# avianphysics/avian

Hardware: NVIDIA H100
Metric: physics steps/sec on 100k-cube stack (broad phase + solver stage per step) (higher is better)
Workload: dtype f32

## Files before the change

avian_b200/csrc/solver_dev.cuh:

```cuda
#pragma once
#include <cuda_pipeline.h>

#include "../../include/avian_b200.h"
#include "avn_math.cuh"

namespace avn {

enum { CP_N = 0, CP_T1 = 1, CP_TV = 2, CP_IDX = 3, CP_PT0 = 4, CP_PLANES = CP_PT0 + 3 * AVN_MAX_MANIFOLD_POINTS };
#define CP_ROW(k, r) (CP_PT0 + 3 * (k) + (r))
enum { CI_NP_MASK = 0x7, CI_ZERO1 = 1 << 4, CI_ZERO2 = 1 << 5, CI_NONDYN = 1 << 6, CI_TANGENT = 1 << 7,
       CI_VER1 = 1 << 8, CI_VER2 = 1 << 9,
       CI_FIV1 = 1 << 10, CI_FIV2 = 1 << 11,
       CI_FIP1 = 1 << 12, CI_FIP2 = 1 << 13 };
enum { BF_LOCK_MASK = 0x3f, BF_HAS_SOLVER_BODY = 1 << 8, BF_KINEMATIC = 1 << 9, BF_GYRO = 1 << 10, BF_DYNAMIC = 1 << 11,
       BF_CUSTOM_VEL = 1 << 12, BF_CUSTOM_POS = 1 << 13, BF_FUSE_IV = 1 << 14, BF_FUSE_IP = 1 << 15, BF_DOMINANCE_SHIFT = 16 };

enum { JP_IDX = 0,
       JP_R1 = 1,
       JP_R2 = 2,
       JP_CD = 3,
       JP_RD = 4,
       JP_A1 = 5,
       JP_A2 = 6,
       JP_B1 = 7,
// ... 193 lines not shown
    {
        S rcp = S(1) / len(tvv);
        if (avn_finite(rcp) && rcp > S(0)) t1 = tvv * rcp; else t1 = any_orthonormal(fd);
    }
    V3<S> t2 = cross(fd, t1);
    S friction = d.m_friction[m], restitution = d.m_restitution[m];
    if (friction > S(0)) info |= CI_TANGENT;
    if (restitution != S(0)) *d.any_restitution = 1;
    V3<S> tv = ldv3_or0(d.m_tanvel, m);
    st4(&c[CP_N * MP], mk4<S>(n.x, n.y, n.z, friction));
    st4(&c[CP_T1 * MP], mk4<S>(t1.x, t1.y, t1.z, restitution));
    st4(&c[CP_TV * MP], mk4<S>(tv.x, tv.y, tv.z, S(0)));
    st4(&c[CP_IDX * MP], mk4<S>(int_as(S(0), b1), int_as(S(0), b2), int_as(S(0), info), int_as(S(0), 0)));
    bool warm = d.match_contacts != 0;
    for (int k = 0; k < np; ++k) {
        uint32_t p = p0 + k;
        V3<S> r1 = ldv3(d.p_anchor1, p), r2 = ldv3(d.p_anchor2, p);
        V3<S> r1xn = cross(r1, n), r2xn = cross(r2, n);
        S k_linear = dot(n, cmul(mass_sum, n));
        S kk = k_linear + dot(r1xn, smul(in1.ii, r1xn)) + dot(r2xn, smul(in2.ii, r2xn));
        S meff = recip_or_zero(kk);
        S sep0 = -d.p_penetration[p] - dot(r2 - r1, n);
        S imp_n = warm ? d.p_ws_normal[p] : S(0);
        S itx = S(0), ity = S(0), K1 = S(0), K2 = S(0), K3 = S(0);
        if (info & CI_TANGENT) {
            if (warm) { itx = d.p_ws_tangent[2 * p]; ity = d.p_ws_tangent[2 * p + 1]; }
            V3<S> rt11 = cross(r1, t1), rt12 = cross(r2, t1), rt21 = cross(r1, t2), rt22 = cross(r2, t2);
            V3<S> i1_rt11 = smul(in1.ii, rt11), i2_rt12 = smul(in2.ii, rt12), i1_rt21 = smul(in1.ii, rt21), i2_rt22 = smul(in2.ii, rt22);
            S kl1 = dot(t1, cmul(mass_sum, t1)), kl2 = dot(t2, cmul(mass_sum, t2));
            K1 = kl1 + dot(rt11, i1_rt11) + dot(rt12, i2_rt12);
            K2 = kl2 + dot(rt21, i1_rt21) + dot(rt22, i2_rt22);
            K3 = S(2) * (dot(rt11, i1_rt21) + dot(rt12, i2_rt22));
        }
        st4(&c[size_t(CP_ROW(k, 0)) * MP], mk4<S>(r1.x, r1.y, r1.z, sep0));
        st4(&c[size_t(CP_ROW(k, 1)) * MP], mk4<S>(r2.x, r2.y, r2.z, meff));
        pc_store(pc_ptr(d, k, slot), mk4<S>(imp_n, S(0), itx, ity));
        st4(&c[size_t(CP_ROW(k, 2)) * MP], mk4<S>(K1, K2, K3, d.p_normal_speed[p]));
    }
}

enum { PASS_WARM = 0, PASS_SOLVE_BIAS = 1, PASS_RELAX = 2, PASS_RESTITUTION = 3 };

template <class S>
__device__ __forceinline__ void apply_impulse(V3<S>& v1, V3<S>& w1, V3<S>& v2, V3<S>& w2, const BodyInertia<S>& in1, const BodyInertia<S>& in2,
                                              V3<S> r1, V3<S> r2, V3<S> imp) {
    v1 = v1 - cmul(imp, in1.inv_mass);
    w1 = w1 - smul(in1.ii, cross(r1, imp));
    v2 = v2 + cmul(imp, in2.inv_mass);
    w2 = w2 + smul(in2.ii, cross(r2, imp));
}

enum { FLAG_RESTITUTION = 0, FLAG_WAVE = 1, FLAG_WORDS = 4 };
#ifdef AVN_WAVE_TRACE
#define AVN_TRACE_T(var) const long long var = clock64()
#define AVN_TRACE_ADD(d, i, v) do { if ((threadIdx.x & 31) == 0) atomicAdd(reinterpret_cast<unsigned long long*>((d).any_restitution + FLAG_WORDS) + (i), (unsigned long long)(v)); } while (0)
#else
#define AVN_TRACE_T(var)
#define AVN_TRACE_ADD(d, i, v)
#endif
__device__ __forceinline__ unsigned events_per_substep(int k, int iters) { return 2u + unsigned(2 + iters) * unsigned(k); }
enum { WV_IV = 0, WV_WARM = 1, WV_SOLVE = 2, WV_IP = 3, WV_RELAX = 4 };
__device__ __forceinline__ unsigned wave_event(int kind, int it, int s, int iters, int k, int r) {
    unsigned base = unsigned(s) * events_per_substep(k, iters);
    switch (kind) {
        case WV_IV: return base;
        case WV_WARM: return base + 1u + r;
        case WV_SOLVE: return base + 1u + unsigned(1 + it) * k + r;
        case WV_IP: return base + 1u + unsigned(1 + iters) * k;
        default: return base + 2u + unsigned(1 + iters) * k + r;
    }
}
__device__ __forceinline__ unsigned ld_acquire(const unsigned* p) {
    unsigned v;
    asm volatile("ld.acquire.gpu.global.u32 %0, [%1];" : "=r"(v) : "l"(p) : "memory");
    return v;
}
__device__ __forceinline__ void st_relaxed(unsigned* p, unsigned v) { asm volatile("st.relaxed.gpu.global.u32 [%0], %1;" ::"l"(p), "r"(v) : "memory"); }
__device__ __forceinline__ void fence_acq_rel() { asm volatile("fence.acq_rel.gpu;" ::: "memory"); }
__device__ __forceinline__ Vec4<float> ld4_cg(const Vec4<float>* p) {
    float4 v = __ldcg(reinterpret_cast<const float4*>(p));
    return mk4<float>(v.x, v.y, v.z, v.w);
}
__device__ __forceinline__ Vec4<double> ld4_cg(const Vec4<double>* p) {
    double2 a = __ldcg(reinterpret_cast<const double2*>(p)), b = __ldcg(reinterpret_cast<const double2*>(p) + 1);
    return mk4<double>(a.x, a.y, b.x, b.y);
}
template <bool WAVE, class S> __device__ __forceinline__ Vec4<S> ldm(const Vec4<S>* p) { return WAVE ? ld4_cg(p) : ld4(p); }
template <bool WAVE, class S> __device__ __forceinline__ Vec4<S> pc_load(const Vec4<S>* p) { return ldm<WAVE>(p); }

template <bool EXACT = true>
__device__ __forceinline__ void wave_wait(const unsigned* ver, bool need1, int b1, unsigned e1, bool need2, int b2, unsigned e2, int* watchdog) {
    for (unsigned spins = 0;; ++spins) {
        if (need1) { const unsigned v = ld_acquire(ver + b1); need1 = EXACT ? v != e1 : v < e1; }
        if (need2) { const unsigned v = ld_acquire(ver + b2); need2 = EXACT ? v != e2 : v < e2; }
        if (__all_sync(0xffffffffu, !(need1 || need2))) break;
        if (spins > (1u << 22)) { *watchdog = 1; break; }
    }
}
__device__ __forceinline__ void wave_publish(unsigned* ver, bool need1, int b1, unsigned e1, bool need2, int b2, unsigned e2, unsigned n1 = 1u,
                                             unsigned n2 = 1u) {
    fence_acq_rel();
    if (need1) st_relaxed(ver + b1, e1 + n1);
    if (need2) st_relaxed(ver + b2, e2 + n2);
}

constexpr int STAGE_ROWS = 3 * AVN_MAX_MANIFOLD_POINTS;
template <class S> __device__ __forceinline__ Vec4<S>* stage_base() {
    extern __shared__ __align__(32) unsigned char avn_stage_raw[];
    return reinterpret_cast<Vec4<S>*>(avn_stage_raw);
}
__device__ __forceinline__ void stage_copy(Vec4<float>* dst, const Vec4<float>* src) { __pipeline_memcpy_async(dst, src, 16); }
__device__ __forceinline__ void stage_copy(Vec4<double>* dst, const Vec4<double>* src) {
    __pipeline_memcpy_async(dst, src, 16);
    __pipeline_memcpy_async(reinterpret_cast<char*>(dst) + 16, reinterpret_cast<const char*>(src) + 16, 16);
}
template <class S> __host__ __device__ constexpr size_t stage_bytes(int threads, int max_points = AVN_MAX_MANIFOLD_POINTS) {
    return size_t(4 * max_points + 1) * threads * sizeof(Vec4<S>);
}

template <class S, int PASS, int MAXP = AVN_MAX_MANIFOLD_POINTS>
__device__ __forceinline__ void contact_item(const DevSolver<S>& d, int slot) {
    const size_t MP = size_t(d.Mpad);
    Vec4<S>* c = d.cst + slot;
    Vec4<S> hidx = ld4(&c[CP_IDX * MP]);
    const int info = as_int(hidx.z);
    const int np = info & CI_NP_MASK;
    if (np == 0) return;
    const int b1 = as_int(hidx.x), b2 = as_int(hidx.y);
    Vec4<S> hn = mk4<S>(0, 0, 0, 0), ht1 = hn, htv = hn;
    BodyInertia<S> in1 = zero_inertia<S>(), in2 = zero_inertia<S>();
    Vec4<S> PC[MAXP];
    constexpr bool SOLVE = (PASS == PASS_SOLVE_BIAS || PASS == PASS_RELAX);
    Vec4<S>* const stage = stage_base<S>() + threadIdx.x;
    const int T = blockDim.x;
#define ROW_A(k) stage[(3 * (k) + 0) * T]
#define ROW_B(k) stage[(3 * (k) + 1) * T]
#define ROW_D(k) stage[(3 * (k) + 2) * T]
    {
        hn = ld4(&c[CP_N * MP]);
        ht1 = ld4(&c[CP_T1 * MP]);
        if (SOLVE) htv = ld4(&c[CP_TV * MP]);
        if (!(info & CI_ZERO1)) in1 = unpack_inertia(ld4(&d.inr[2 * b1]), ld4(&d.inr[2 * b1 + 1]));
        if (!(info & CI_ZERO2)) in2 = unpack_inertia(ld4(&d.inr[2 * b2]), ld4(&d.inr[2 * b2 + 1]));
#pragma unroll
        for (int k = 0; k < MAXP; ++k) {
            if (k < np) {
                stage_copy(&ROW_A(k), &c[size_t(CP_ROW(k, 0)) * MP]);
                stage_copy(&ROW_B(k), &c[size_t(CP_ROW(k, 1)) * MP]);
                if (PASS == PASS_RESTITUTION || (SOLVE && (info & CI_TANGENT))) stage_copy(&ROW_D(k), &c[size_t(CP_ROW(k, 2)) * MP]);
            }
        }
    }
    __pipeline_commit();
    Vec4<S> l1 = ld4(&d.vel[2 * b1]), a1 = ld4(&d.vel[2 * b1 + 1]);
    Vec4<S> l2 = ld4(&d.vel[2 * b2]), a2 = ld4(&d.vel[2 * b2 + 1]);
    Vec4<S> dp1, dq1, dp2, dq2;
// ... 132 lines not shown
__device__ __forceinline__ void wave_contact_item(const DevSolver<S>& d, int slot, int s, int it, bool lane_active, bool relax) {
    constexpr bool SOLVE = PASS == PASS_SOLVE_BIAS;
    relax = SOLVE && relax;
    const size_t MP = size_t(d.Mpad);
    const Vec4<S>* c = d.cst + (lane_active ? slot : 0);
    const Vec4<S> hidx = ld4(&c[CP_IDX * MP]);
    const int info = lane_active ? as_int(hidx.z) : 0;
    const int np = info & CI_NP_MASK;
    const int b1 = as_int(hidx.x), b2 = as_int(hidx.y);
    Vec4<S>* const stage = stage_base<S>() + threadIdx.x;
    const int T = blockDim.x;
#define ROW_A(k) stage[(3 * (k) + 0) * T]
#define ROW_B(k) stage[(3 * (k) + 1) * T]
#define ROW_D(k) stage[(3 * (k) + 2) * T]
#define ROW_PC(k) stage[(3 * MAXP + (k)) * T]
    S* const sepv = reinterpret_cast<S*>(&stage[(4 * MAXP) * T]);
    Vec4<S> hn = mk4<S>(0, 0, 0, 0), ht1 = hn, htv = hn;
    BodyInertia<S> in1 = zero_inertia<S>(), in2 = zero_inertia<S>();
    if (np != 0) {
        hn = ld4(&c[CP_N * MP]);
        ht1 = ld4(&c[CP_T1 * MP]);
        if (SOLVE) htv = ld4(&c[CP_TV * MP]);
        if (!(info & CI_ZERO1)) in1 = unpack_inertia(ld4(&d.inr[2 * b1]), ld4(&d.inr[2 * b1 + 1]));
        if (!(info & CI_ZERO2)) in2 = unpack_inertia(ld4(&d.inr[2 * b2]), ld4(&d.inr[2 * b2 + 1]));
#pragma unroll 1
        for (int k = 0; k < np; ++k) {
            stage_copy(&ROW_A(k), &c[size_t(CP_ROW(k, 0)) * MP]);
            stage_copy(&ROW_B(k), &c[size_t(CP_ROW(k, 1)) * MP]);
            if (SOLVE && (info & CI_TANGENT)) stage_copy(&ROW_D(k), &c[size_t(CP_ROW(k, 2)) * MP]);
        }
    }
    __pipeline_commit();
    const bool ver1 = np != 0 && (info & CI_VER1), ver2 = np != 0 && (info & CI_VER2);
    const int rk = as_int(hidx.w);
    const int k1 = (rk >> 8) & 0xff, k2 = (rk >> 24) & 0xff;
    const int kind = SOLVE ? (relax ? WV_RELAX : WV_SOLVE) : WV_WARM;
    const unsigned e1 = wave_event(kind, it, s, d.iters, k1, rk & 0xff);
    const unsigned e2 = wave_event(kind, it, s, d.iters, k2, (rk >> 16) & 0xff);
#ifdef AVN_FUSE_IV
    const bool fiv1 = relax && (info & CI_FIV1) && s + 1 < d.substeps, fiv2 = relax && (info & CI_FIV2) && s + 1 < d.substeps;
#else
    constexpr bool fiv1 = false, fiv2 = false;
#endif
#ifdef AVN_FUSE_IP
    const bool fip1 = SOLVE && !relax && (info & CI_FIP1) && it + 1 == d.iters, fip2 = SOLVE && !relax && (info & CI_FIP2) && it + 1 == d.iters;
#else
    constexpr bool fip1 = false, fip2 = false;
#endif
    Vec4<S> il1, ia1, il2, ia2;
    if (fiv1) { il1 = ld4(&d.itg[2 * b1]); ia1 = ld4(&d.itg[2 * b1 + 1]); }
    if (fiv2) { il2 = ld4(&d.itg[2 * b2]); ia2 = ld4(&d.itg[2 * b2 + 1]); }
    int* const watchdog = d.any_restitution + FLAG_WAVE;
    const V3<S> n = xyz(hn), t1 = xyz(ht1);

    if (SOLVE) {
        AVN_TRACE_T(t_d0);
        const int sd = relax ? s : s - 1;
        if (sd >= 0)
            wave_wait<false>(d.ver, ver1, b1, wave_event(WV_IP, 0, sd, d.iters, k1, 0) + 1u, ver2, b2, wave_event(WV_IP, 0, sd, d.iters, k2, 0) + 1u,
                             watchdog);
        __pipeline_wait_prior(0);
        if (np != 0) {
            const Vec4<S> dp1 = ld4_cg(&d.dlt[2 * b1]), dq1 = ld4_cg(&d.dlt[2 * b1 + 1]);
            const Vec4<S> dp2 = ld4_cg(&d.dlt[2 * b2]), dq2 = ld4_cg(&d.dlt[2 * b2 + 1]);
            Q4<S> q1; q1.x = dq1.x; q1.y = dq1.y; q1.z = dq1.z; q1.w = dq1.w;
            Q4<S> q2; q2.x = dq2.x; q2.y = dq2.y; q2.z = dq2.z; q2.w = dq2.w;
            const V3<S> delta_translation = xyz(dp2) - xyz(dp1);
#pragma unroll 1
            for (int k = 0; k < np; ++k) {
                const Vec4<S> PAk = ROW_A(k), PBk = ROW_B(k);
                V3<S> rr1 = qrot(q1, xyz(PAk)), rr2 = qrot(q2, xyz(PBk));
                V3<S> dsep = delta_translation + (rr2 - rr1);
                sepv[k] = dot(dsep, n) + PAk.w;
            }
        }
#ifdef AVN_WAVE_TRACE
        if (np != 0 && sepv[0] == S(1.2345e33)) d.any_restitution[1] = 2;
        AVN_TRACE_ADD(d, 5, clock64() - t_d0);
#endif
    }

    AVN_TRACE_T(t_w0);
    wave_wait(d.ver, ver1, b1, e1, ver2, b2, e2, watchdog);
    AVN_TRACE_ADD(d, 0, clock64() - t_w0);
    if (np == 0) return;
    AVN_TRACE_T(t_l0);
    const Vec4<S> l1 = ld4_cg(&d.vel[2 * b1]), a1 = ld4_cg(&d.vel[2 * b1 + 1]);
    const Vec4<S> l2 = ld4_cg(&d.vel[2 * b2]), a2 = ld4_cg(&d.vel[2 * b2 + 1]);
    {
        Vec4<S> pc[MAXP];
#pragma unroll
        for (int k = 0; k < MAXP; ++k)
            if (k < np) pc[k] = pc_load<true>(pc_ptr(d, k, slot));
#pragma unroll
        for (int k = 0; k < MAXP; ++k)
            if (k < np) ROW_PC(k) = pc[k];
    }
    if (!SOLVE) __pipeline_wait_prior(0);
#ifdef AVN_WAVE_TRACE
    if ((l1.x + a1.x + l2.x + a2.x) == S(1.2345e33)) d.any_restitution[1] = 2;
    AVN_TRACE_T(t_c0);
    AVN_TRACE_ADD(d, 1, t_c0 - t_l0);
#endif
    V3<S> v1 = xyz(l1), w1 = xyz(a1), v2 = xyz(l2), w2 = xyz(a2);
    const V3<S> t2 = cross(t1, n);

    if (!SOLVE) {
#pragma unroll 1
        for (int k = 0; k < np; ++k) {
            const Vec4<S> PAk = ROW_A(k), PBk = ROW_B(k), pck = ROW_PC(k);
            V3<S> r1 = xyz(PAk), r2 = xyz(PBk);
            S tx = (info & CI_TANGENT) ? pck.z : S(0), ty = (info & CI_TANGENT) ? pck.w : S(0);
            V3<S> p = d.warm_coeff * ((pck.x * n + tx * t1) + ty * t2);
            apply_impulse(v1, w1, v2, w2, in1, in2, r1, r2, p);
        }
    } else {
        const Soft<S> soft = (info & CI_NONDYN) ? d.soft_nondyn : d.soft_dyn;
#pragma unroll 1
        for (int k = 0; k < np; ++k) {
            const Vec4<S> PAk = ROW_A(k), PBk = ROW_B(k);
            Vec4<S> pck = ROW_PC(k);
            V3<S> r1 = xyz(PAk), r2 = xyz(PBk);
            const S separation = sepv[k];
            V3<S> relv = (v2 + cross(w2, r2)) - (v1 + cross(w1, r1));
            S vn = dot(relv, n);
            S meff = PBk.w, acc = pck.x;
            S impulse;
            if (separation > S(0)) {
                impulse = -meff * (vn + separation / d.h);
            } else if (!relax) {
                S bias = avn_max(soft.bias * separation, -d.max_overlap_speed);
                S scaled_mass = soft.mass_scale * meff;
                S scaled_impulse = soft.impulse_scale * acc;
                impulse = -scaled_mass * (vn + bias) - scaled_impulse;
            } else {
                impulse = -meff * vn;
            }
            S new_impulse = avn_max(acc + impulse, S(0));
            impulse = new_impulse - acc;
            pck.x = new_impulse;
            pck.y = pck.y + new_impulse;
            ROW_PC(k) = pck;
            apply_impulse(v1, w1, v2, w2, in1, in2, r1, r2, impulse * n);
        }
        if (info & CI_TANGENT) {
            const S friction = hn.w;
            const V3<S> surf = xyz(htv);
#pragma unroll 1
            for (int k = 0; k < np; ++k) {
                const Vec4<S> PAk = ROW_A(k), PBk = ROW_B(k), PDk = ROW_D(k);
                Vec4<S> pck = ROW_PC(k);
                V3<S> r1 = xyz(PAk), r2 = xyz(PBk);
                V3<S> relv = (v2 + cross(w2, r2)) - (v1 + cross(w1, r1));
                S limit = friction * pck.x;
                relv = relv + surf;
                S ts1 = dot(relv, t1), ts2 = dot(relv, t2);
                S t11 = ts1 * ts1, t22 = ts2 * ts2, t12 = ts1 * ts2;
                S inv = (t11 * PDk.x + t22 * PDk.y) + t12 * PDk.z;
                S em = (t11 + t22) * (S(1) / inv);
                V3<S> imp = zero3<S>();
                if (avn_finite(em)) {
                    S nx = pck.z - em * ts1, ny = pck.w - em * ts2;
                    S l2 = nx * nx + ny * ny;
                    if (l2 > limit * limit) {
                        S l = avn_sqrt(l2);
                        nx = limit * (nx / l);
                        ny = limit * (ny / l);
                    }
                    S dx = nx - pck.z, dy = ny - pck.w;
                    pck.z = nx;
                    pck.w = ny;
                    ROW_PC(k) = pck;
                    imp = dx * t1 + dy * t2;
                }
                apply_impulse(v1, w1, v2, w2, in1, in2, r1, r2, imp);
            }
        }
    }
#ifdef AVN_WAVE_TRACE
    if ((v1.x + v2.x + w1.x + w2.x) == S(1.2345e33)) d.any_restitution[1] = 2;
    AVN_TRACE_T(t_s0);
    AVN_TRACE_ADD(d, 2, t_s0 - t_c0);
#endif
    if (SOLVE) {
#pragma unroll 1
        for (int k = 0; k < np; ++k) pc_store(pc_ptr(d, k, slot), ROW_PC(k));
    }
    if (fip1) {
        const Vec4<S> dp = ld4_cg(&d.dlt[2 * b1]), dq4 = ld4_cg(&d.dlt[2 * b1 + 1]);
        V3<S> ndp = xyz(dp) + v1 * d.h;
        Q4<S> q; q.x = dq4.x; q.y = dq4.y; q.z = dq4.z; q.w = dq4.w;
        Q4<S> nq = qmul(q_from_scaled_axis(w1 * d.h, d.fast_trig != 0), q);
        st4(&d.dlt[2 * b1], mk4<S>(ndp.x, ndp.y, ndp.z, S(0)));
        st4(&d.dlt[2 * b1 + 1], mk4<S>(nq.x, nq.y, nq.z, nq.w));
    }
    if (fip2) {
        const Vec4<S> dp = ld4_cg(&d.dlt[2 * b2]), dq4 = ld4_cg(&d.dlt[2 * b2 + 1]);
        V3<S> ndp = xyz(dp) + v2 * d.h;
        Q4<S> q; q.x = dq4.x; q.y = dq4.y; q.z = dq4.z; q.w = dq4.w;
        Q4<S> nq = qmul(q_from_scaled_axis(w2 * d.h, d.fast_trig != 0), q);
        st4(&d.dlt[2 * b2], mk4<S>(ndp.x, ndp.y, ndp.z, S(0)));
        st4(&d.dlt[2 * b2 + 1], mk4<S>(nq.x, nq.y, nq.z, nq.w));
    }
    if (fiv1) { v1 = v1 * il1.w; w1 = w1 * ia1.w; v1 = v1 + xyz(il1); w1 = w1 + xyz(ia1); }
    if (fiv2) { v2 = v2 * il2.w; w2 = w2 * ia2.w; v2 = v2 + xyz(il2); w2 = w2 + xyz(ia2); }
    if (!(info & CI_ZERO1) || fiv1) {
        st4(&d.vel[2 * b1], mk4<S>(v1.x, v1.y, v1.z, S(0)));
        st4(&d.vel[2 * b1 + 1], mk4<S>(w1.x, w1.y, w1.z, S(0)));
    }
    if (!(info & CI_ZERO2) || fiv2) {
        st4(&d.vel[2 * b2], mk4<S>(v2.x, v2.y, v2.z, S(0)));
        st4(&d.vel[2 * b2 + 1], mk4<S>(w2.x, w2.y, w2.z, S(0)));
    }
    wave_publish(d.ver, ver1, b1, e1, ver2, b2, e2, (fiv1 || fip1) ? 2u : 1u, (fiv2 || fip2) ? 2u : 1u);
#ifdef AVN_WAVE_TRACE
    AVN_TRACE_ADD(d, 3, clock64() - t_s0);
    AVN_TRACE_ADD(d, 4, 1);
#endif
#undef ROW_A
#undef ROW_B
#undef ROW_D
#undef ROW_PC
}

template <class S, bool WAVE = false>
__device__ __forceinline__ void integrate_velocity_item(const DevSolver<S>& d, int i, int s = 0, bool lane_active = true) {
    const bool in_range = lane_active && i < d.B;
    int f = 0;
    if (in_range) f = as_int(ld4(&d.inr[2 * i]).y);
    bool live = in_range && (f & BF_HAS_SOLVER_BODY);
    if (WAVE && live && (f & BF_FUSE_IV) && s >= 1 && d.deg[i] > 0) live = false;
    unsigned e = 0;
    if (WAVE) {
        if (live) e = wave_event(WV_IV, 0, s, d.iters, d.deg[i], 0);
        wave_wait(d.ver, live, i, e, false, 0, 0u, d.any_restitution + 1);
    }
    if (!live) return;
    Vec4<S> l = ldm<WAVE>(&d.vel[2 * i]), a = ldm<WAVE>(&d.vel[2 * i + 1]);
    V3<S> v = xyz(l), w = xyz(a);
    bool touched = false;
    if (!(f & BF_CUSTOM_VEL) && !(f & BF_KINEMATIC)) {
        Vec4<S> li = ld4(&d.itg[2 * i]), ai = ld4(&d.itg[2 * i + 1]);
        v = v * li.w;
        w = w * ai.w;
        v = v + xyz(li);
        w = w + xyz(ai);
        if (f & BF_GYRO) {
            Vec4<S> dq4 = ldm<WAVE>(&d.dlt[2 * i + 1]);
            Q4<S> dq; dq.x = dq4.x; dq.y = dq4.y; dq.z = dq4.z; dq.w = dq4.w;
            Q4<S> rot = qmul(dq, ldq(d.rotation, i));
            Sym3<S> il;
            il.m00 = d.inv_inertia_local[6 * i]; il.m01 = d.inv_inertia_local[6 * i + 1]; il.m02 = d.inv_inertia_local[6 * i + 2];
            il.m11 = d.inv_inertia_local[6 * i + 3]; il.m12 = d.inv_inertia_local[6 * i + 4]; il.m22 = d.inv_inertia_local[6 * i + 5];
            V3<S> lw = qrot(qconj(rot), w);
            Sym3<S> tensor = sym_inverse_or_zero(il);
            V3<S> L = smul(tensor, lw);
            V3<S> Ln = L - d.h * cross(lw, L);
            S l2 = len2(Ln);
            if (l2 == S(0)) {
                w = zero3<S>();
            } else {
                Ln = Ln * avn_sqrt(len2(L) / l2);
                w = qrot(rot, smul(il, Ln));
            }
        }
        touched = true;
    }
    if (d.max_lin) {
        S ms = d.max_lin[i];
// ... 144 lines not shown
```

avian_b200/csrc/solver_host.cu:

```cuda
#include <algorithm>
#include <cmath>
#include <cstdlib>
#include <cstring>

#include "context.hpp"
#include "joint_schedule.hpp"
#include "island_lists.hpp"
#include "solver_kernels.cuh"

namespace avn {

namespace {

template <class S>
Soft<S> softness(S damping_ratio, S hz, S delta_secs) {
    S double_damping_ratio = S(2) * damping_ratio;
    S angular_frequency = S(6.283185307179586476925286766559) * hz;
    S a1 = double_damping_ratio + angular_frequency * delta_secs;
    S a2 = angular_frequency * delta_secs * a1;
    S a3 = S(1) / (S(1) + a2);
    Soft<S> s;
    s.bias = angular_frequency / a1;
    s.mass_scale = a2 * a3;
    s.impulse_scale = a3;
// ... 930 lines not shown
        if ((st = comm->all_reduce_max_i32(bnd_agree_.as<int>(), 1)) != AVN_OK) return st;
        AVN_CUDA(cudaMemcpyAsync(h_agree_, bnd_agree_.p, sizeof(int), cudaMemcpyDeviceToHost, stream_));
        AVN_CUDA(cudaStreamSynchronize(stream_));
        any_rest = *h_agree_;
        agreed_rest_ = any_rest;
        agreed_valid_ = true;
    }
    const uint32_t substeps = uint32_t(dev_.substeps);
    for (uint32_t s = 0; s < substeps; ++s) {
        if ((st = run_range(s, 1, s == 0 ? AVN_RUN_PREPARE : 0u)) != AVN_OK) return st;
        if ((st = exchange()) != AVN_OK) return st;
    }
    if (substeps == 0 && (st = run_range(0, 0, AVN_RUN_PREPARE)) != AVN_OK) return st;
    if (any_rest) {
        if ((st = boundary_snapshot()) != AVN_OK) return st;
        if ((st = run_range(substeps, 0, AVN_RUN_RESTITUTION)) != AVN_OK) return st;
        if ((st = exchange()) != AVN_OK) return st;
    }
    return run_range(substeps, 0, AVN_RUN_FINALIZE);
}

template <class S>
AvnStatus Solver<S>::download() {
    if (!ran_) return err_->fail(AVN_ERR_INVALID_ARGUMENT, "avn_solver_download before avn_solver_run");
    const size_t B = hb_.count;
    cudaEventRecord(ev_[EV_D2H0], stream_);
    if (B) {
        AVN_CUDA(cudaMemcpyAsync(hb_.position, dev_.out_position, 3 * B * sizeof(S), cudaMemcpyDeviceToHost, stream_));
        AVN_CUDA(cudaMemcpyAsync(hb_.rotation, dev_.out_rotation, 4 * B * sizeof(S), cudaMemcpyDeviceToHost, stream_));
        AVN_CUDA(cudaMemcpyAsync(hb_.linear_velocity, dev_.out_linvel, 3 * B * sizeof(S), cudaMemcpyDeviceToHost, stream_));
        AVN_CUDA(cudaMemcpyAsync(hb_.angular_velocity, dev_.out_angvel, 3 * B * sizeof(S), cudaMemcpyDeviceToHost, stream_));
    }
    if (have_m_ && !hm_.device) {
        const size_t P = hm_.P;
        AVN_CUDA(cudaMemcpyAsync(hm_.ws_normal, dev_.p_out_ws_normal, P * sizeof(S), cudaMemcpyDeviceToHost, stream_));
        AVN_CUDA(cudaMemcpyAsync(hm_.ws_tangent, dev_.p_out_ws_tangent, 2 * P * sizeof(S), cudaMemcpyDeviceToHost, stream_));
        AVN_CUDA(cudaMemcpyAsync(hm_.normal_impulse, dev_.p_normal_impulse, P * sizeof(S), cudaMemcpyDeviceToHost, stream_));
    }
    if (have_j_) {
        for (int t = 0; t < AVN_JOINT_TYPE_COUNT; ++t) {
            const size_t n = hj_.types[t].count;
            if (n && dev_.jforce[t]) AVN_CUDA(cudaMemcpyAsync(hj_.types[t].force, dev_.jforce[t], 3 * n * sizeof(S), cudaMemcpyDeviceToHost, stream_));
            if (n && dev_.jtorque[t]) AVN_CUDA(cudaMemcpyAsync(hj_.types[t].torque, dev_.jtorque[t], 3 * n * sizeof(S), cudaMemcpyDeviceToHost, stream_));
        }
    }
    int flags_host[2] = {0, 0};
    AVN_CUDA(cudaMemcpyAsync(flags_host, dev_.any_restitution, sizeof flags_host, cudaMemcpyDeviceToHost, stream_));
    cudaEventRecord(ev_[EV_D2H1], stream_);
    AVN_CUDA(cudaStreamSynchronize(stream_));
#ifdef AVN_WAVE_TRACE
    {
        unsigned long long tr[8];
        cudaMemcpy(tr, dev_.any_restitution + FLAG_WORDS, sizeof tr, cudaMemcpyDeviceToHost);
        if (tr[4]) fprintf(stderr, "[avn wave trace] contact item-warps %llu  avg cycles: stage 1 (wait deltas + separations) %.0f  wait %.0f  loads %.0f  compute %.0f  "
                           "store+publish %.0f\n", tr[4], double(tr[5]) / tr[4], double(tr[0]) / tr[4], double(tr[1]) / tr[4], double(tr[2]) / tr[4], double(tr[3]) / tr[4]);
    }
#endif
    if (flags_host[1] == WAVE_BAD_COLOURING)
        return err_->fail(AVN_ERR_INVALID_ARGUMENT, "manifolds: invalid colouring — a body with a SolverBody appears twice in one graph colour (or carries more than 254 "
                                                    "constraints): the colours are not conflict-free, the results of this step are not reliable");
    if (flags_host[1] == WAVE_WATCHDOG) return err_->fail(AVN_ERR_CUDA, "wavefront scheduler watchdog fired: results are invalid (set AVN_LAUNCH_MODE=barrier)");
    float ms = 0;
    if (cudaEventElapsedTime(&ms, ev_[EV_H2D0], ev_[EV_H2D1]) == cudaSuccess) tm_.h2d_ms = ms;
    if (cudaEventElapsedTime(&ms, ev_[EV_RUN0], ev_[EV_PREP]) == cudaSuccess) tm_.prepare_ms = ms;
    if (cudaEventElapsedTime(&ms, ev_[EV_PREP], ev_[EV_LOOP]) == cudaSuccess) tm_.substep_loop_ms = ms;
    if (cudaEventElapsedTime(&ms, ev_[EV_LOOP], ev_[EV_RUN1]) == cudaSuccess) tm_.finalize_ms = ms;
    if (cudaEventElapsedTime(&ms, ev_[EV_D2H0], ev_[EV_D2H1]) == cudaSuccess) tm_.d2h_ms = ms;
    if (cudaEventElapsedTime(&ms, ev_[EV_RUN0], ev_[EV_RUN1]) == cudaSuccess) tm_.total_ms = ms;
    tm_.kernel_launches = launches_;
    tm_.contact_constraint_count = uint32_t(dev_.M);
    tm_.joint_levels = uint32_t(dev_.n_levels);
    uint32_t ac = 0;
    for (int c = 0; c < AVN_GRAPH_COLOR_COUNT; ++c) ac += dev_.color_len[c] > 0;
    tm_.active_colors = ac;
    tm_.launch_mode = !mega_step_ ? AVN_LAUNCH_PHASES : (dev_.wave ? AVN_LAUNCH_MEGA_WAVE : (dev_.isl_count > 0 ? AVN_LAUNCH_MEGA_ISLANDS : AVN_LAUNCH_MEGA_BARRIER));
    return AVN_OK;
}

}

SolverBase* make_solver(uint32_t scalar_bits, cudaStream_t stream, ErrorSink* err, uint32_t cfg_flags, int device) {
    if (scalar_bits == 32) return new Solver<float>(stream, err, cfg_flags, device);
    if (scalar_bits == 64) return new Solver<double>(stream, err, cfg_flags, device);
    return nullptr;
}

}
```

avian_b200/csrc/solver_kernels.cuh:

```cuda
#pragma once
#include <cooperative_groups.h>

#include "joints_dev.cuh"

namespace avn {
namespace cg = cooperative_groups;

constexpr int MEGA_BLOCK = 128;

enum PhaseOp {
    OP_PREPARE_BODY = 0, OP_PREPARE_CONSTRAINT, OP_PREPARE_JOINT, OP_INTEGRATE_VEL, OP_INTEGRATE_POS, OP_WARM, OP_SOLVE_BIAS,
    OP_RELAX, OP_RESTITUTION, OP_SOLVE_JOINT, OP_PROJECT_VEL, OP_DAMP_JOINT, OP_WRITEBACK_BODY, OP_STORE_IMPULSE, OP_JOINT_FORCE,
    OP_WAVE_RANK, OP_WAVE_PACK
};

template <class S, int OP, int MAXP = AVN_MAX_MANIFOLD_POINTS>
__device__ __forceinline__ void run_item(const DevSolver<S>& d, int i) {
    if (OP == OP_PREPARE_BODY) prepare_body_item(d, i);
    else if (OP == OP_PREPARE_CONSTRAINT) prepare_constraint_item(d, i);
    else if (OP == OP_PREPARE_JOINT) prepare_joint_item(d, i);
    else if (OP == OP_INTEGRATE_VEL) integrate_velocity_item(d, i);
    else if (OP == OP_INTEGRATE_POS) { integrate_position_item(d, i); if (d.J > 0) store_pre_solve_item(d, i); }
    else if (OP == OP_WARM) contact_item<S, PASS_WARM, MAXP>(d, i);
    else if (OP == OP_SOLVE_BIAS) contact_item<S, PASS_SOLVE_BIAS, MAXP>(d, i);
// ... 39 lines not shown
    for (int c = 0; c < AVN_COLOR_OVERFLOW; ++c) {
        const int b = d.color_off[c], n = d.color_len[c];
        if (n <= 0) continue;
        grid_phase<S, OP, MAXP>(d, b, n);
        grid.sync();
    }
}

#ifndef AVN_WAVE_CHUNK
#define AVN_WAVE_CHUNK 32
#endif
constexpr int WAVE_CHUNK = AVN_WAVE_CHUNK;
template <class S, int PASS, int MAXP, int BPS>
__device__ __noinline__ void wave_contact_chunk(const DevSolver<S>& d, int slot, int s, int it, bool active, bool relax) {
    wave_contact_item<S, PASS, MAXP>(d, slot, s, it, active, relax);
}
template <class S, int BPS, int MAXP>
__device__ __noinline__ void wave_iv_chunk(const DevSolver<S>& d, int i, int s, bool active) { integrate_velocity_item<S, true>(d, i, s, active); }
template <class S, int BPS, int MAXP>
__device__ __noinline__ void wave_ip_chunk(const DevSolver<S>& d, int i, int s, bool active) { integrate_position_item<S, true>(d, i, s, active); }

template <class S, int MAXP>
__device__ __forceinline__ void wave_prefetch_slot(const DevSolver<S>& d, int slot) {
#ifdef AVN_WAVE_PREFETCH
    const char* base = reinterpret_cast<const char*>(d.cst + slot);
    const size_t stride = size_t(d.Mpad) * sizeof(Vec4<S>);
#pragma unroll
    for (int r = 0; r < CP_PT0 + 3 * MAXP; ++r) asm volatile("prefetch.global.L2 [%0];" ::"l"(base + size_t(r) * stride));
#endif
}

template <class S, int MAXP, int BPS>
__device__ __forceinline__ void wave_substep_loop(const DevSolver<S>& d) {
    const int lane = threadIdx.x & 31;
    const bool active = lane < WAVE_CHUNK;
    const long long warps = (long long)gridDim.x * (blockDim.x >> 5);
    long long warp_id = (long long)blockIdx.x * (blockDim.x >> 5) + (threadIdx.x >> 5);
    if (d.sm_slots) {
        __shared__ int ticket, dense;
        unsigned smid;
        asm volatile("mov.u32 %0, %%smid;" : "=r"(smid));
        if (threadIdx.x == 0) {
            const int t = atomicAdd(&d.sm_slots[smid & 255u], 1);
            ticket = t % BPS;
            int* slot = &d.sm_slots[256 + (smid & 255u)];
            if (ticket == 0 && atomicAdd(slot, 0) == 0) atomicExch(slot, atomicAdd(&d.sm_slots[512], 1) + 1);
            int v;
            while ((v = atomicAdd(slot, 0)) == 0) { }
            dense = v - 1;
        }
        __syncthreads();
        warp_id = ((long long)dense * BPS + ticket) * (blockDim.x >> 5) + (threadIdx.x >> 5);
    }
    const int body_chunks = (d.B + WAVE_CHUNK - 1) / WAVE_CHUNK, slot_chunks = d.Mpad / WAVE_CHUNK;
    const int first_chunks = body_chunks;
    const int front_passes = 1 + d.iters;
    const long long per_substep = (long long)first_chunks + body_chunks + (long long)(front_passes + 1) * slot_chunks;
    const long long total = per_substep * d.sub_end;
    [[maybe_unused]] auto contact_slot_of = [&](long long r) -> int {
        if (r < first_chunks) return -1;
        r -= first_chunks;
        if (r < (long long)front_passes * slot_chunks) return int(r % slot_chunks) * WAVE_CHUNK;
        r -= (long long)front_passes * slot_chunks;
        if (r < body_chunks) return -1;
        return int(r - body_chunks) * WAVE_CHUNK;
    };
    for (long long g = per_substep * d.sub_begin + warp_id; g < total; g += warps) {
        const int s = int(g / per_substep);
        long long r = g - (long long)s * per_substep;
#ifdef AVN_WAVE_PREFETCH
        {
            const long long gn = g + warps;
            if (gn < total) {
                const int ns = contact_slot_of(gn % per_substep);
                if (ns >= 0 && active) wave_prefetch_slot<S, MAXP>(d, ns + lane);
            }
        }
#endif
        if (r < first_chunks) {
            wave_iv_chunk<S, BPS, MAXP>(d, int(r) * WAVE_CHUNK + lane, s, active);
            continue;
        }
        r -= first_chunks;
        if (r < (long long)front_passes * slot_chunks) {
            const int pass = int(r / slot_chunks), slot = int(r - (long long)pass * slot_chunks) * WAVE_CHUNK + lane;
            if (pass == 0) wave_contact_chunk<S, PASS_WARM, MAXP, BPS>(d, slot, s, 0, active, false);
            else wave_contact_chunk<S, PASS_SOLVE_BIAS, MAXP, BPS>(d, slot, s, pass - 1, active, false);
            continue;
        }
        r -= (long long)front_passes * slot_chunks;
        if (r < body_chunks) { wave_ip_chunk<S, BPS, MAXP>(d, int(r) * WAVE_CHUNK + lane, s, active); continue; }
        r -= body_chunks;
        wave_contact_chunk<S, PASS_SOLVE_BIAS, MAXP, BPS>(d, int(r) * WAVE_CHUNK + lane, s, 0, active, true);
    }
}

template <class S, int OP, int MAXP>
__device__ __noinline__ void island_phase(const DevSolver<S>& d, const int* __restrict__ list, int lo, int hi) {
    for (int k = lo + int(threadIdx.x); k < hi; k += int(blockDim.x)) run_item<S, OP, MAXP>(d, list[k]);
    __syncthreads();
}
template <class S, int OP, int MAXP>
__device__ __forceinline__ void island_contact_pass(const DevSolver<S>& d, int isl) {
    const int* off = d.isl_m_off + size_t(isl) * (AVN_GRAPH_COLOR_COUNT + 1);
    for (int c = 0; c < AVN_COLOR_OVERFLOW; ++c) {
        const int lo = off[c], hi = off[c + 1];
        if (hi > lo) island_phase<S, OP, MAXP>(d, d.isl_mslots, lo, hi);
    }
}
template <class S, int MAXP>
__device__ __forceinline__ void island_substep_loop(const DevSolver<S>& d) {
    for (int isl = int(blockIdx.x); isl < d.isl_count; isl += int(gridDim.x)) {
        const int b0 = d.isl_body_off[isl], b1 = d.isl_body_off[isl + 1];
        const int* joff = d.isl_j_off + size_t(isl) * (d.isl_levels + 1);
        const bool has_m = d.M > 0 && d.isl_m_off[size_t(isl) * (AVN_GRAPH_COLOR_COUNT + 1)] < d.isl_m_off[size_t(isl) * (AVN_GRAPH_COLOR_COUNT + 1) + AVN_GRAPH_COLOR_COUNT];
        for (int sub = d.sub_begin; sub < d.sub_end; ++sub) {
            island_phase<S, OP_INTEGRATE_VEL, MAXP>(d, d.isl_bodies, b0, b1);
            if (has_m) {
                island_contact_pass<S, OP_WARM, MAXP>(d, isl);
                for (int it = 0; it < d.iters; ++it) island_contact_pass<S, OP_SOLVE_BIAS, MAXP>(d, isl);
            }
            island_phase<S, OP_INTEGRATE_POS, MAXP>(d, d.isl_bodies, b0, b1);
            if (has_m) island_contact_pass<S, OP_RELAX, MAXP>(d, isl);
            if (d.J > 0) {
                for (int l = 0; l < d.isl_levels; ++l)
                    if (joff[l + 1] > joff[l]) island_phase<S, OP_SOLVE_JOINT, MAXP>(d, d.isl_jslots, joff[l], joff[l + 1]);
                island_phase<S, OP_PROJECT_VEL, MAXP>(d, d.isl_bodies, b0, b1);
                if (d.any_joint_damping)
                    for (int l = 0; l < d.isl_levels; ++l)
                        if (joff[l + 1] > joff[l]) island_phase<S, OP_DAMP_JOINT, MAXP>(d, d.isl_jslots, joff[l], joff[l + 1]);
            }
        }
    }
}

template <class S, int BPS, int MAXP>
__global__ void __launch_bounds__(MEGA_BLOCK, BPS) step_megakernel(const __grid_constant__ DevSolver<S> d) {
    cg::grid_group grid = cg::this_grid();
    if (d.do_prepare) {
        grid_phase<S, OP_PREPARE_BODY>(d, 0, d.B + 1);
        grid.sync();
        grid_phase<S, OP_PREPARE_CONSTRAINT>(d, 0, d.M);
        grid_phase<S, OP_PREPARE_JOINT>(d, 0, d.J);
        grid.sync();
        if (d.wave) {
            for (int c = 0; c < AVN_COLOR_OVERFLOW; ++c) {
                if (d.color_len[c] <= 0) continue;
// ... 54 lines not shown
```

Baseline: 420.5.

## Split acquire/release fences, hoist impulse loads, pad wave segments to warp multiples

Replaces the acquire loads in the wave spin-wait with relaxed loads followed by a single acquire fence, and replaces the acq_rel fence before publishing with a release fence. Impulse loads and warm-start impulse computation are hoisted ahead of the dependency wait so they overlap the spin. Accumulated impulse stores now happen after publishing the version counters, taking them off the critical path. Each phase segment of the persistent work schedule is padded to a multiple of the warp count so every warp keeps a fixed phase slot. The padding adds idle iterations, and the relaxed ordering depends on the fences being placed correctly. Trace counters are moved to shared-memory accumulators.

```diff
diff --git a/avian_b200/csrc/solver_dev.cuh b/avian_b200/csrc/solver_dev.cuh
--- a/avian_b200/csrc/solver_dev.cuh
+++ b/avian_b200/csrc/solver_dev.cuh
@@ -269,8 +269,9 @@
 
 enum { FLAG_RESTITUTION = 0, FLAG_WAVE = 1, FLAG_WORDS = 4 };
 #ifdef AVN_WAVE_TRACE
+__device__ __forceinline__ unsigned long long* avn_trace_acc() { __shared__ unsigned long long acc[8]; return acc; }
 #define AVN_TRACE_T(var) const long long var = clock64()
-#define AVN_TRACE_ADD(d, i, v) do { if ((threadIdx.x & 31) == 0) atomicAdd(reinterpret_cast<unsigned long long*>((d).any_restitution + FLAG_WORDS) + (i), (unsigned long long)(v)); } while (0)
+#define AVN_TRACE_ADD(d, i, v) do { if ((threadIdx.x & 31) == 0) atomicAdd(avn_trace_acc() + (i), (unsigned long long)(v)); } while (0)
 #else
 #define AVN_TRACE_T(var)
 #define AVN_TRACE_ADD(d, i, v)
@@ -287,13 +288,14 @@
         default: return base + 2u + unsigned(1 + iters) * k + r;
     }
 }
-__device__ __forceinline__ unsigned ld_acquire(const unsigned* p) {
+__device__ __forceinline__ unsigned ld_relaxed(const unsigned* p) {
     unsigned v;
-    asm volatile("ld.acquire.gpu.global.u32 %0, [%1];" : "=r"(v) : "l"(p) : "memory");
+    asm volatile("ld.relaxed.gpu.global.u32 %0, [%1];" : "=r"(v) : "l"(p) : "memory");
     return v;
 }
 __device__ __forceinline__ void st_relaxed(unsigned* p, unsigned v) { asm volatile("st.relaxed.gpu.global.u32 [%0], %1;" ::"l"(p), "r"(v) : "memory"); }
-__device__ __forceinline__ void fence_acq_rel() { asm volatile("fence.acq_rel.gpu;" ::: "memory"); }
+__device__ __forceinline__ void fence_acquire() { asm volatile("fence.acquire.gpu;" ::: "memory"); }
+__device__ __forceinline__ void fence_release() { asm volatile("fence.release.gpu;" ::: "memory"); }
 __device__ __forceinline__ Vec4<float> ld4_cg(const Vec4<float>* p) {
     float4 v = __ldcg(reinterpret_cast<const float4*>(p));
     return mk4<float>(v.x, v.y, v.z, v.w);
@@ -308,17 +310,22 @@
 template <bool EXACT = true>
 __device__ __forceinline__ void wave_wait(const unsigned* ver, bool need1, int b1, unsigned e1, bool need2, int b2, unsigned e2, int* watchdog) {
     for (unsigned spins = 0;; ++spins) {
-        if (need1) { const unsigned v = ld_acquire(ver + b1); need1 = EXACT ? v != e1 : v < e1; }
-        if (need2) { const unsigned v = ld_acquire(ver + b2); need2 = EXACT ? v != e2 : v < e2; }
+        if (need1) { const unsigned v = ld_relaxed(ver + b1); need1 = EXACT ? v != e1 : v < e1; }
+        if (need2) { const unsigned v = ld_relaxed(ver + b2); need2 = EXACT ? v != e2 : v < e2; }
         if (__all_sync(0xffffffffu, !(need1 || need2))) break;
         if (spins > (1u << 22)) { *watchdog = 1; break; }
     }
+    fence_acquire();
+}
+__device__ __forceinline__ void wave_publish_counters(unsigned* ver, bool need1, int b1, unsigned e1, bool need2, int b2, unsigned e2,
+                                                      unsigned n1 = 1u, unsigned n2 = 1u) {
+    if (need1) st_relaxed(ver + b1, e1 + n1);
+    if (need2) st_relaxed(ver + b2, e2 + n2);
 }
 __device__ __forceinline__ void wave_publish(unsigned* ver, bool need1, int b1, unsigned e1, bool need2, int b2, unsigned e2, unsigned n1 = 1u,
                                              unsigned n2 = 1u) {
-    fence_acq_rel();
-    if (need1) st_relaxed(ver + b1, e1 + n1);
-    if (need2) st_relaxed(ver + b2, e2 + n2);
+    fence_release();
+    wave_publish_counters(ver, need1, b1, e1, need2, b2, e2, n1, n2);
 }
 
 constexpr int STAGE_ROWS = 3 * AVN_MAX_MANIFOLD_POINTS;
@@ -557,9 +564,29 @@
     if (fiv2) { il2 = ld4(&d.itg[2 * b2]); ia2 = ld4(&d.itg[2 * b2 + 1]); }
     int* const watchdog = d.any_restitution + FLAG_WAVE;
     const V3<S> n = xyz(hn), t1 = xyz(ht1);
-
+    const V3<S> t2 = cross(t1, n);
+
+    AVN_TRACE_T(t_d0);
+    Vec4<S> pc[MAXP];
+    if (np != 0) {
+#pragma unroll
+        for (int k = 0; k < MAXP; ++k)
+            if (k < np) pc[k] = pc_load<true>(pc_ptr(d, k, slot));
+        if (!SOLVE) {
+#pragma unroll
+            for (int k = 0; k < MAXP; ++k) {
+                if (k >= np) continue;
+                S tx = (info & CI_TANGENT) ? pc[k].z : S(0), ty = (info & CI_TANGENT) ? pc[k].w : S(0);
+                V3<S> p = d.warm_coeff * ((pc[k].x * n + tx * t1) + ty * t2);
+                ROW_PC(k) = mk4<S>(p.x, p.y, p.z, S(0));
+            }
+        }
+    }
+
+#ifdef AVN_WAVE_TRACE
+    long long t_d1 = t_d0;
+#endif
     if (SOLVE) {
-        AVN_TRACE_T(t_d0);
         const int sd = relax ? s : s - 1;
         if (sd >= 0)
             wave_wait<false>(d.ver, ver1, b1, wave_event(WV_IP, 0, sd, d.iters, k1, 0) + 1u, ver2, b2, wave_event(WV_IP, 0, sd, d.iters, k2, 0) + 1u,
@@ -568,6 +595,9 @@
         if (np != 0) {
             const Vec4<S> dp1 = ld4_cg(&d.dlt[2 * b1]), dq1 = ld4_cg(&d.dlt[2 * b1 + 1]);
             const Vec4<S> dp2 = ld4_cg(&d.dlt[2 * b2]), dq2 = ld4_cg(&d.dlt[2 * b2 + 1]);
+#pragma unroll
+            for (int k = 0; k < MAXP; ++k)
+                if (k < np) ROW_PC(k) = pc[k];
             Q4<S> q1; q1.x = dq1.x; q1.y = dq1.y; q1.z = dq1.z; q1.w = dq1.w;
             Q4<S> q2; q2.x = dq2.x; q2.y = dq2.y; q2.z = dq2.z; q2.w = dq2.w;
             const V3<S> delta_translation = xyz(dp2) - xyz(dp1);
@@ -581,43 +611,28 @@
         }
 #ifdef AVN_WAVE_TRACE
         if (np != 0 && sepv[0] == S(1.2345e33)) d.any_restitution[1] = 2;
-        AVN_TRACE_ADD(d, 5, clock64() - t_d0);
+        t_d1 = clock64();
 #endif
     }
 
     AVN_TRACE_T(t_w0);
     wave_wait(d.ver, ver1, b1, e1, ver2, b2, e2, watchdog);
-    AVN_TRACE_ADD(d, 0, clock64() - t_w0);
     if (np == 0) return;
     AVN_TRACE_T(t_l0);
     const Vec4<S> l1 = ld4_cg(&d.vel[2 * b1]), a1 = ld4_cg(&d.vel[2 * b1 + 1]);
     const Vec4<S> l2 = ld4_cg(&d.vel[2 * b2]), a2 = ld4_cg(&d.vel[2 * b2 + 1]);
-    {
-        Vec4<S> pc[MAXP];
-#pragma unroll
-        for (int k = 0; k < MAXP; ++k)
-            if (k < np) pc[k] = pc_load<true>(pc_ptr(d, k, slot));
-#pragma unroll
-        for (int k = 0; k < MAXP; ++k)
-            if (k < np) ROW_PC(k) = pc[k];
-    }
     if (!SOLVE) __pipeline_wait_prior(0);
 #ifdef AVN_WAVE_TRACE
     if ((l1.x + a1.x + l2.x + a2.x) == S(1.2345e33)) d.any_restitution[1] = 2;
     AVN_TRACE_T(t_c0);
-    AVN_TRACE_ADD(d, 1, t_c0 - t_l0);
 #endif
     V3<S> v1 = xyz(l1), w1 = xyz(a1), v2 = xyz(l2), w2 = xyz(a2);
-    const V3<S> t2 = cross(t1, n);
 
     if (!SOLVE) {
 #pragma unroll 1
         for (int k = 0; k < np; ++k) {
-            const Vec4<S> PAk = ROW_A(k), PBk = ROW_B(k), pck = ROW_PC(k);
-            V3<S> r1 = xyz(PAk), r2 = xyz(PBk);
-            S tx = (info & CI_TANGENT) ? pck.z : S(0), ty = (info & CI_TANGENT) ? pck.w : S(0);
-            V3<S> p = d.warm_coeff * ((pck.x * n + tx * t1) + ty * t2);
-            apply_impulse(v1, w1, v2, w2, in1, in2, r1, r2, p);
+            const Vec4<S> PAk = ROW_A(k), PBk = ROW_B(k);
+            apply_impulse(v1, w1, v2, w2, in1, in2, xyz(PAk), xyz(PBk), xyz(ROW_PC(k)));
         }
     } else {
         const Soft<S> soft = (info & CI_NONDYN) ? d.soft_nondyn : d.soft_dyn;
@@ -685,12 +700,7 @@
 #ifdef AVN_WAVE_TRACE
     if ((v1.x + v2.x + w1.x + w2.x) == S(1.2345e33)) d.any_restitution[1] = 2;
     AVN_TRACE_T(t_s0);
-    AVN_TRACE_ADD(d, 2, t_s0 - t_c0);
 #endif
-    if (SOLVE) {
-#pragma unroll 1
-        for (int k = 0; k < np; ++k) pc_store(pc_ptr(d, k, slot), ROW_PC(k));
-    }
     if (fip1) {
         const Vec4<S> dp = ld4_cg(&d.dlt[2 * b1]), dq4 = ld4_cg(&d.dlt[2 * b1 + 1]);
         V3<S> ndp = xyz(dp) + v1 * d.h;
@@ -717,9 +727,23 @@
         st4(&d.vel[2 * b2], mk4<S>(v2.x, v2.y, v2.z, S(0)));
         st4(&d.vel[2 * b2 + 1], mk4<S>(w2.x, w2.y, w2.z, S(0)));
     }
-    wave_publish(d.ver, ver1, b1, e1, ver2, b2, e2, (fiv1 || fip1) ? 2u : 1u, (fiv2 || fip2) ? 2u : 1u);
+    AVN_TRACE_T(t_f0);
+    fence_release();
+    AVN_TRACE_T(t_f1);
+    wave_publish_counters(d.ver, ver1, b1, e1, ver2, b2, e2, (fiv1 || fip1) ? 2u : 1u, (fiv2 || fip2) ? 2u : 1u);
+    if (SOLVE) {
+#pragma unroll 1
+        for (int k = 0; k < np; ++k) pc_store(pc_ptr(d, k, slot), ROW_PC(k));
+    }
 #ifdef AVN_WAVE_TRACE
-    AVN_TRACE_ADD(d, 3, clock64() - t_s0);
+    const long long t_e = clock64();
+    if (SOLVE) AVN_TRACE_ADD(d, 5, t_d1 - t_d0);
+    AVN_TRACE_ADD(d, 0, t_l0 - t_w0);
+    AVN_TRACE_ADD(d, 1, t_c0 - t_l0);
+    AVN_TRACE_ADD(d, 2, t_s0 - t_c0);
+    AVN_TRACE_ADD(d, 3, t_f0 - t_s0);
+    AVN_TRACE_ADD(d, 6, t_f1 - t_f0);
+    AVN_TRACE_ADD(d, 7, t_e - t_f1);
     AVN_TRACE_ADD(d, 4, 1);
 #endif
 #undef ROW_A
diff --git a/avian_b200/csrc/solver_host.cu b/avian_b200/csrc/solver_host.cu
--- a/avian_b200/csrc/solver_host.cu
+++ b/avian_b200/csrc/solver_host.cu
@@ -1006,8 +1006,10 @@
     {
         unsigned long long tr[8];
         cudaMemcpy(tr, dev_.any_restitution + FLAG_WORDS, sizeof tr, cudaMemcpyDeviceToHost);
-        if (tr[4]) fprintf(stderr, "[avn wave trace] contact item-warps %llu  avg cycles: stage 1 (wait deltas + separations) %.0f  wait %.0f  loads %.0f  compute %.0f  "
-                           "store+publish %.0f\n", tr[4], double(tr[5]) / tr[4], double(tr[0]) / tr[4], double(tr[1]) / tr[4], double(tr[2]) / tr[4], double(tr[3]) / tr[4]);
+        if (tr[4]) fprintf(stderr, "[avn wave trace] contact item-warps %llu  avg cycles: stage 1 (impulse loads + wait deltas + separations) %.0f  wait %.0f  "
+                           "loads %.0f  compute %.0f  store issue %.0f  fence %.0f  counters+impulses %.0f\n", tr[4], double(tr[5]) / tr[4],
+                           double(tr[0]) / tr[4], double(tr[1]) / tr[4], double(tr[2]) / tr[4], double(tr[3]) / tr[4], double(tr[6]) / tr[4],
+                           double(tr[7]) / tr[4]);
     }
 #endif
     if (flags_host[1] == WAVE_BAD_COLOURING)
diff --git a/avian_b200/csrc/solver_kernels.cuh b/avian_b200/csrc/solver_kernels.cuh
--- a/avian_b200/csrc/solver_kernels.cuh
+++ b/avian_b200/csrc/solver_kernels.cuh
@@ -115,18 +115,22 @@
         __syncthreads();
         warp_id = ((long long)dense * BPS + ticket) * (blockDim.x >> 5) + (threadIdx.x >> 5);
     }
+#ifdef AVN_WAVE_TRACE
+    if (threadIdx.x < 8) avn_trace_acc()[threadIdx.x] = 0;
+    __syncthreads();
+#endif
     const int body_chunks = (d.B + WAVE_CHUNK - 1) / WAVE_CHUNK, slot_chunks = d.Mpad / WAVE_CHUNK;
-    const int first_chunks = body_chunks;
+    const long long body_seg = (body_chunks + warps - 1) / warps * warps, slot_seg = (slot_chunks + warps - 1) / warps * warps;
     const int front_passes = 1 + d.iters;
-    const long long per_substep = (long long)first_chunks + body_chunks + (long long)(front_passes + 1) * slot_chunks;
+    const long long per_substep = 2 * body_seg + (long long)(front_passes + 1) * slot_seg;
     const long long total = per_substep * d.sub_end;
     [[maybe_unused]] auto contact_slot_of = [&](long long r) -> int {
-        if (r < first_chunks) return -1;
-        r -= first_chunks;
-        if (r < (long long)front_passes * slot_chunks) return int(r % slot_chunks) * WAVE_CHUNK;
-        r -= (long long)front_passes * slot_chunks;
-        if (r < body_chunks) return -1;
-        return int(r - body_chunks) * WAVE_CHUNK;
+        if (r < body_seg) return -1;
+        r -= body_seg;
+        if (r < (long long)front_passes * slot_seg) r %= slot_seg;
+        else if ((r -= (long long)front_passes * slot_seg) < body_seg) return -1;
+        else r -= body_seg;
+        return r < slot_chunks ? int(r) * WAVE_CHUNK : -1;
     };
     for (long long g = per_substep * d.sub_begin + warp_id; g < total; g += warps) {
         const int s = int(g / per_substep);
@@ -140,22 +144,30 @@
             }
         }
 #endif
-        if (r < first_chunks) {
-            wave_iv_chunk<S, BPS, MAXP>(d, int(r) * WAVE_CHUNK + lane, s, active);
+        if (r < body_seg) {
+            if (r < body_chunks) wave_iv_chunk<S, BPS, MAXP>(d, int(r) * WAVE_CHUNK + lane, s, active);
             continue;
         }
-        r -= first_chunks;
-        if (r < (long long)front_passes * slot_chunks) {
-            const int pass = int(r / slot_chunks), slot = int(r - (long long)pass * slot_chunks) * WAVE_CHUNK + lane;
-            if (pass == 0) wave_contact_chunk<S, PASS_WARM, MAXP, BPS>(d, slot, s, 0, active, false);
-            else wave_contact_chunk<S, PASS_SOLVE_BIAS, MAXP, BPS>(d, slot, s, pass - 1, active, false);
+        r -= body_seg;
+        if (r < (long long)front_passes * slot_seg) {
+            const int pass = int(r / slot_seg), q = int(r - (long long)pass * slot_seg);
+            if (q >= slot_chunks) continue;
+            if (pass == 0) wave_contact_chunk<S, PASS_WARM, MAXP, BPS>(d, q * WAVE_CHUNK + lane, s, 0, active, false);
+            else wave_contact_chunk<S, PASS_SOLVE_BIAS, MAXP, BPS>(d, q * WAVE_CHUNK + lane, s, pass - 1, active, false);
             continue;
         }
-        r -= (long long)front_passes * slot_chunks;
-        if (r < body_chunks) { wave_ip_chunk<S, BPS, MAXP>(d, int(r) * WAVE_CHUNK + lane, s, active); continue; }
-        r -= body_chunks;
-        wave_contact_chunk<S, PASS_SOLVE_BIAS, MAXP, BPS>(d, int(r) * WAVE_CHUNK + lane, s, 0, active, true);
-    }
+        r -= (long long)front_passes * slot_seg;
+        if (r < body_seg) {
+            if (r < body_chunks) wave_ip_chunk<S, BPS, MAXP>(d, int(r) * WAVE_CHUNK + lane, s, active);
+            continue;
+        }
+        r -= body_seg;
+        if (r < slot_chunks) wave_contact_chunk<S, PASS_SOLVE_BIAS, MAXP, BPS>(d, int(r) * WAVE_CHUNK + lane, s, 0, active, true);
+    }
+#ifdef AVN_WAVE_TRACE
+    __syncthreads();
+    if (threadIdx.x < 8) atomicAdd(reinterpret_cast<unsigned long long*>(d.any_restitution + FLAG_WORDS) + threadIdx.x, avn_trace_acc()[threadIdx.x]);
+#endif
 }
 
 template <class S, int OP, int MAXP>
```

Measured after the change: 431.5, median of 6. 1.03x the previous value.
